# david-strejc/fei

Hardware: AMD Instinct MI355X
Metric: agent tok/s (llama3-8b local decode, 1 agent/GPU) (higher is better)
Workload: dtype bf16; 1 GPU; model=llama3-8b, global_batch=1, seq_len=512, parallelism=dp1 (1 agent per GPU, weak scaling), hip_graph=True, stream_engine=False

## Files before the change

fei_amd/models/llama.py:

```python

from __future__ import annotations

import math
import os
from dataclasses import dataclass
from typing import Dict, List, Optional

import torch
import torch.nn.functional as F

from fei_amd import ops
from fei_amd.engine.config import ModelSpec
from fei_amd.ops import reference as ref
from fei_amd.parallel.pg import ParallelContext, all_gather_cat, all_reduce_sum


@dataclass
class LayerWeights:
    norm_attn: torch.Tensor
    wqkv: torch.Tensor
    wo: torch.Tensor
    norm_mlp: torch.Tensor
    wgu: torch.Tensor
    wdown: torch.Tensor
# ... 16 lines not shown
        self.max_seq_len = max_seq_len or spec.max_seq_len
        tp_size = self.tp.world_size if self.tp.is_distributed else 1
        if spec.num_kv_heads % tp_size or spec.num_heads % tp_size or \
                spec.intermediate_size % tp_size or spec.vocab_size % tp_size:
            raise ValueError(f"model {spec.name} not divisible by tp={tp_size}")
        self.tp_size = tp_size
        self.tp_rank = self.tp.rank if self.tp.is_distributed else 0
        self.hq_l = spec.num_heads // tp_size
        self.hkv_l = spec.num_kv_heads // tp_size
        self.inter_l = spec.intermediate_size // tp_size
        self.vocab_l = spec.vocab_size // tp_size
        self.D = spec.head_dim
        self._init_weights(seed)
        self.rope = ref.rope_table(self.max_seq_len, self.D, spec.rope_theta,
                                   device=device)
        self.prefetch_mb = int(os.environ.get("FEI_PREFETCH", "0") or 0)
        self._pf_stream = None
        self._pf_sink = None
        self.norm_precomp = os.environ.get("FEI_NORM_PRECOMP", "0") == "1"


    def _rand(self, gen, *shape, scale: float) -> torch.Tensor:
        w = torch.randn(*shape, generator=gen, device=self.device,
                        dtype=torch.float32) * scale
        return w.to(self.dtype)

    def _init_weights(self, seed: int) -> None:
        s = self.spec
        gen = torch.Generator(device=self.device)
        gen.manual_seed(seed)
        C = s.hidden_size
        sc = 1.0 / math.sqrt(C)
        self.emb = self._rand(gen, s.vocab_size, C, scale=0.02)
        self.layers: List[LayerWeights] = []
        r = self.tp_rank
        for _ in range(s.num_layers):
            wq = self._rand(gen, s.num_heads * self.D, C, scale=sc)
            wk = self._rand(gen, s.num_kv_heads * self.D, C, scale=sc)
            wv = self._rand(gen, s.num_kv_heads * self.D, C, scale=sc)
            wo = self._rand(gen, C, s.num_heads * self.D, scale=sc / math.sqrt(2 * s.num_layers))
            wg = self._rand(gen, s.intermediate_size, C, scale=sc)
            wu = self._rand(gen, s.intermediate_size, C, scale=sc)
            wd = self._rand(gen, C, s.intermediate_size,
                            scale=1.0 / math.sqrt(s.intermediate_size) / math.sqrt(2 * s.num_layers))
            wq = wq.view(s.num_heads, self.D, C)[r * self.hq_l:(r + 1) * self.hq_l].reshape(-1, C)
            wk = wk.view(s.num_kv_heads, self.D, C)[r * self.hkv_l:(r + 1) * self.hkv_l].reshape(-1, C)
            wv = wv.view(s.num_kv_heads, self.D, C)[r * self.hkv_l:(r + 1) * self.hkv_l].reshape(-1, C)
            wo = wo.view(C, s.num_heads, self.D)[:, r * self.hq_l:(r + 1) * self.hq_l].reshape(C, -1)
            wg = wg[r * self.inter_l:(r + 1) * self.inter_l]
            wu = wu[r * self.inter_l:(r + 1) * self.inter_l]
            wd = wd[:, r * self.inter_l:(r + 1) * self.inter_l]
            self.layers.append(LayerWeights(
                norm_attn=torch.ones(C, device=self.device, dtype=self.dtype),
                wqkv=torch.cat([wq, wk, wv], dim=0).contiguous(),
                wo=wo.contiguous(),
                norm_mlp=torch.ones(C, device=self.device, dtype=self.dtype),
                wgu=torch.cat([wg, wu], dim=0).contiguous(),
                wdown=wd.contiguous(),
            ))
        self.norm_f = torch.ones(C, device=self.device, dtype=self.dtype)
        lm = self._rand(gen, s.vocab_size, C, scale=sc)
        self.lm_head = lm[r * self.vocab_l:(r + 1) * self.vocab_l].contiguous()
        self.vocab_offset = r * self.vocab_l

    def quantize_fp8(self) -> None:
        self.fp8 = []
        for lw in self.layers:
            self.fp8.append({
                "wqkv": ops.quant_fp8(lw.wqkv),
                "wo": ops.quant_fp8(lw.wo),
                "wgu": ops.quant_fp8(lw.wgu),
                "wdown": ops.quant_fp8(lw.wdown),
            })
        self.fp8_lm_head = ops.quant_fp8(self.lm_head)

    def param_bytes(self) -> int:
        total = self.emb.numel() + self.norm_f.numel() + self.lm_head.numel()
        for lw in self.layers:
            for t in (lw.norm_attn, lw.wqkv, lw.wo, lw.norm_mlp, lw.wgu, lw.wdown):
                total += t.numel()
        return total * self.emb.element_size()


    def new_kv_cache(self, batch: int, max_seq: Optional[int] = None,
                     kv_quant: Optional[str] = None):
        max_seq = max_seq or self.max_seq_len
        shape = (batch, self.hkv_l, max_seq, self.D)
        if kv_quant == "fp8":
            return (
                [ops.QuantKV.zeros(shape, self.device)
                 for _ in range(self.spec.num_layers)],
                [ops.QuantKV.zeros(shape, self.device)
                 for _ in range(self.spec.num_layers)],
            )
        if kv_quant is not None:
            raise ValueError(f"unknown kv_quant {kv_quant!r}")
        return (
            [torch.zeros(shape, device=self.device, dtype=self.dtype)
             for _ in range(self.spec.num_layers)],
            [torch.zeros(shape, device=self.device, dtype=self.dtype)
             for _ in range(self.spec.num_layers)],
        )


    def _qkv_views(self, qkv: torch.Tensor, B: int, S: Optional[int] = None):
        D = self.D
        W = qkv.shape[-1]
        off_k = self.hq_l * D
        off_v = off_k + self.hkv_l * D
        if S is None:
            q = qkv.as_strided((B, self.hq_l, D), (W, D, 1))
            k = qkv.as_strided((B, self.hkv_l, D), (W, D, 1), storage_offset=qkv.storage_offset() + off_k)
            v = qkv.as_strided((B, self.hkv_l, D), (W, D, 1), storage_offset=qkv.storage_offset() + off_v)
        else:
            q = qkv.as_strided((B, S, self.hq_l, D), (S * W, W, D, 1))
            k = qkv.as_strided((B, S, self.hkv_l, D), (S * W, W, D, 1), storage_offset=qkv.storage_offset() + off_k)
            v = qkv.as_strided((B, S, self.hkv_l, D), (S * W, W, D, 1), storage_offset=qkv.storage_offset() + off_v)
        return q, k, v


    def forward_decode(
        self,
        token: torch.Tensor,
        pos: torch.Tensor,
        k_caches: List[torch.Tensor],
        v_caches: List[torch.Tensor],
        attn_splits: int = 32,
        workspace=None,
        fused_attn: bool = False,
        attn_out: Optional[torch.Tensor] = None,
        fused_norm: bool = False,
        gather_logits: bool = True,
    ) -> torch.Tensor:
        if fused_norm and self.tp_size == 1 and token.shape[0] == 1 and \
                self.spec.hidden_size * 2 <= 32 * 1024:
            return self._forward_decode_fused_norm(
                token, pos, k_caches, v_caches, attn_splits, workspace,
                fused_attn, attn_out)
        s = self.spec
        B = token.shape[0]
        h = F.embedding(token.long(), self.emb)
        scale = 1.0 / math.sqrt(self.D)
        n_layers = len(self.layers)
        x = ops.rmsnorm(h, self.layers[0].norm_attn, s.norm_eps)
        addnorm = (ops._ADDNORM_GEMV and self.tp_size == 1 and B == 1
                   and h.is_cuda and h.dtype == torch.bfloat16
                   and ops._addnorm_ok(B, s.hidden_size))
        if addnorm:
            h = h.contiguous()
            hb = torch.empty(2, B, s.hidden_size, dtype=h.dtype,
                             device=h.device)
            nbuf = 0
        d = None
        for li, lw in enumerate(self.layers):
            if addnorm and li > 0:
                qkv = ops.gemv_addnorm(d, h, hb[nbuf], lw.norm_attn, lw.wqkv,
                                       s.norm_eps)
                h, nbuf = hb[nbuf], nbuf ^ 1
            else:
                qkv = ops.linear_decode(x, lw.wqkv)
            q, k, v = self._qkv_views(qkv, B)
            if fused_attn:
                att = ops.attn_decode_fused(q, k, v, k_caches[li],
                                            v_caches[li], pos, self.rope,
                                            scale=scale, out=attn_out)
            else:
                att = ops.attn_decode(q, k_caches[li], v_caches[li], pos,
                                      splits=attn_splits, scale=scale,
                                      workspace=workspace, out=attn_out,
                                      k=k, v=v, table=self.rope, layer=li)
            o = ops.linear_decode(att.reshape(B, -1), lw.wo)
            all_reduce_sum(o, self.tp)
            if addnorm:
                act = ops.gemv_swiglu_addnorm(o, h, hb[nbuf], lw.norm_mlp,
                                              lw.wgu, s.norm_eps)
                h, nbuf = hb[nbuf], nbuf ^ 1
            else:
                x, h = ops.fused_add_rmsnorm(o, h, lw.norm_mlp, s.norm_eps)
                act = ops.gemv_swiglu(x, lw.wgu)
            d = ops.linear_decode(act, lw.wdown)
            all_reduce_sum(d, self.tp)
            if addnorm and li + 1 < n_layers:
                continue
            next_norm = (self.layers[li + 1].norm_attn if li + 1 < n_layers
                         else self.norm_f)
            x, h = ops.fused_add_rmsnorm(d, h, next_norm, s.norm_eps)
        logits = ops.linear_decode(x, self.lm_head)
        if gather_logits:
            logits = all_gather_cat(logits, dim=-1, ctx=self.tp)
        return logits

    def forward_decode_stream(self, token, pos, k_caches, v_caches,
                              ws: dict, bufs) -> torch.Tensor:
        s = self.spec
        h = F.embedding(token.long(), self.emb)
        bufs[0].copy_(h.to(bufs[0].dtype))
        scale = 1.0 / math.sqrt(self.D)
        cur, nxt = bufs
        for li, lw in enumerate(self.layers):
            ops.stream_layer(cur, nxt, lw, s, k_caches[li], v_caches[li],
                             self.rope, pos, ws, li, scale)
            cur, nxt = nxt, cur
        return ops.gemv_norm(cur, self.norm_f, self.lm_head, s.norm_eps)

    def _ssq_slots(self, B: int, device) -> torch.Tensor:
        buf = getattr(self, "_ssq", None)
        if buf is None or buf.shape[1] != B or buf.device != device:
            buf = torch.zeros(2 * len(self.layers), B, dtype=torch.float32,
                              device=device)
            self._ssq = buf
        return buf

    def _forward_decode_fused_norm(self, token, pos, k_caches, v_caches,
                                   attn_splits, workspace, fused_attn,
                                   attn_out):
        s = self.spec
        B = token.shape[0]
        fp8 = getattr(self, "fp8", None)
        if fp8 is not None and (B != 1 or s.hidden_size * 2 > 32 * 1024):
            fp8 = None
        h = F.embedding(token.long(), self.emb).contiguous()
        scale = 1.0 / math.sqrt(self.D)
        ssq = (self._ssq_slots(B, h.device)
               if (self.norm_precomp and fp8 is None and h.is_cuda) else None)
        if ssq is not None:
            ssq.zero_()
        pf = self.prefetch_mb > 0 and fp8 is None and h.is_cuda
        if pf and self._pf_stream is None:
            self._pf_stream = torch.cuda.Stream()
            self._pf_sink = torch.zeros(1, dtype=torch.float32,
                                        device=h.device)
        for li, lw in enumerate(self.layers):
            if fp8 is not None:
                q8 = fp8[li]
                qkv = ops.gemv_norm_fp8(h, lw.norm_attn, *q8["wqkv"],
                                        s.norm_eps)
            else:
                qkv = ops.gemv_norm(
                    h, lw.norm_attn, lw.wqkv, s.norm_eps,
                    ssq=ssq[2 * li - 1] if (ssq is not None and li > 0) else None)
            if pf:
                ev = torch.cuda.Event()
                ev.record()
                with torch.cuda.stream(self._pf_stream):
                    self._pf_stream.wait_event(ev)
                    ops.prefetch(lw.wgu, self.prefetch_mb << 20,
                                 self._pf_sink)
            q, k, v = self._qkv_views(qkv, B)
            if fused_attn:
                att = ops.attn_decode_fused(q, k, v, k_caches[li],
                                            v_caches[li], pos, self.rope,
                                            scale=scale, out=attn_out)
            else:
                att = ops.attn_decode(q, k_caches[li], v_caches[li], pos,
                                      splits=attn_splits, scale=scale,
                                      workspace=workspace, out=attn_out,
                                      k=k, v=v, table=self.rope, layer=li)
            if fp8 is not None:
                ops.gemv_res_fp8(att.reshape(B, -1), *q8["wo"], h)
                act = ops.gemv_swiglu_norm_fp8(h, lw.norm_mlp, *q8["wgu"],
                                               s.norm_eps)
                ops.gemv_res_fp8(act, *q8["wdown"], h)
            else:
                ops.gemv_res(att.reshape(B, -1), lw.wo, h,
                             ssq_out=ssq[2 * li] if ssq is not None else None)
                act = ops.gemv_swiglu_norm(
                    h, lw.norm_mlp, lw.wgu, s.norm_eps,
                    ssq=ssq[2 * li] if ssq is not None else None)
                ops.gemv_res(act, lw.wdown, h,
                             ssq_out=ssq[2 * li + 1] if ssq is not None else None)
        if pf:
            torch.cuda.current_stream().wait_stream(self._pf_stream)
        if fp8 is not None:
            return ops.gemv_norm_fp8(h, self.norm_f, *self.fp8_lm_head,
                                     s.norm_eps)
        return ops.gemv_norm(h, self.norm_f, self.lm_head, s.norm_eps,
                             ssq=ssq[-1] if ssq is not None else None)

    def forward_prefill(
        self,
        tokens: torch.Tensor,
        pos0: torch.Tensor,
        k_caches: List[torch.Tensor],
        v_caches: List[torch.Tensor],
        all_positions: bool = False,
    ) -> torch.Tensor:
        scale = 1.0 / math.sqrt(self.D)

        def attend(li, q, k, v):
            ops.rope_kv_prefill(q, k, v, k_caches[li], v_caches[li], pos0, self.rope)
            return ops.attn_prefill(q, k_caches[li], v_caches[li], pos0, scale=scale)

        return self._prefill_layers(tokens, attend, all_positions)

    def forward_prefill_paged(
        self,
        tokens: torch.Tensor,
        pos0: torch.Tensor,
        k_pools: List[torch.Tensor],
        v_pools: List[torch.Tensor],
        block_table: torch.Tensor,
        all_positions: bool = False,
    ) -> torch.Tensor:
        if self.tp_size != 1:
            raise RuntimeError("forward_prefill_paged is single-GPU (tp=1)")
        scale = 1.0 / math.sqrt(self.D)

        def attend(li, q, k, v):
            ops.rope_kv_prefill_paged(q, k, v, k_pools[li], v_pools[li],
                                      block_table, pos0, self.rope)
            return ops.attn_prefill_paged(q, k_pools[li], v_pools[li],
                                          block_table, pos0, scale=scale)

        return self._prefill_layers(tokens, attend, all_positions)

    def _prefill_layers(self, tokens, attend, all_positions):
        s = self.spec
        B, S = tokens.shape
        h = F.embedding(tokens.long(), self.emb)
        n_layers = len(self.layers)
        x = ops.rmsnorm(h, self.layers[0].norm_attn, s.norm_eps)
        for li, lw in enumerate(self.layers):
            qkv = F.linear(x, lw.wqkv)
            qkv2 = qkv.view(B * S, -1)
            q, k, v = self._qkv_views(qkv2, B, S)
            att = attend(li, q, k, v)
            o = F.linear(att.reshape(B, S, -1), lw.wo)
            all_reduce_sum(o, self.tp)
            x, h = ops.fused_add_rmsnorm(o, h, lw.norm_mlp, s.norm_eps)
            gu = F.linear(x, lw.wgu)
            act = ops.swiglu(gu)
            d = F.linear(act, lw.wdown)
            all_reduce_sum(d, self.tp)
            next_norm = (self.layers[li + 1].norm_attn if li + 1 < n_layers
                         else self.norm_f)
            x, h = ops.fused_add_rmsnorm(d, h, next_norm, s.norm_eps)
        last = x if all_positions else x[:, -1, :]
        logits = F.linear(last, self.lm_head)
        logits = all_gather_cat(logits, dim=-1, ctx=self.tp)
        return logits
# ... 70 lines not shown
```

fei_amd/ops/__init__.py:

```python

from __future__ import annotations

import ctypes
import math
import os
from typing import Optional, Tuple

import torch

from fei_amd.ops import reference as ref

_LIB: Optional[ctypes.CDLL] = None
_LIB_ERR: Optional[str] = None
_LIB_PATH = os.path.join(os.path.dirname(os.path.abspath(__file__)),
                         "libfei_kernels.so")

_c = ctypes
_vp, _i, _f, _u64, _l = _c.c_void_p, _c.c_int, _c.c_float, _c.c_ulonglong, _c.c_long


def _try_load() -> None:
    global _LIB, _LIB_ERR
    if _LIB is not None or _LIB_ERR is not None:
        return
    try:
        lib = ctypes.CDLL(_LIB_PATH)
    except OSError as e:
        _LIB_ERR = str(e)
        return
    lib.fei_rmsnorm.argtypes = [_vp, _vp, _vp, _i, _i, _f, _vp]
    lib.fei_add_rmsnorm.argtypes = [_vp, _vp, _vp, _vp, _i, _i, _f, _vp]
    lib.fei_rope_kv_decode.argtypes = [_vp, _vp, _vp, _vp, _vp, _vp, _vp,
                                       _i, _i, _i, _i, _i, _l, _l, _vp]
    lib.fei_rope_kv_prefill.argtypes = [_vp, _vp, _vp, _vp, _vp, _vp, _vp,
                                        _i, _i, _i, _i, _i, _i, _l, _l, _vp]
    lib.fei_attn_decode.argtypes = [_vp, _vp, _vp, _vp, _vp, _vp,
                                    _i, _i, _i, _i, _i, _i, _f, _l,
                                    _vp, _vp, _vp, _l, _vp, _vp, _i, _vp]
    lib.fei_attn_decode_combine.argtypes = [_vp, _vp, _vp, _i, _i, _i, _i, _vp]
    lib.fei_swiglu.argtypes = [_vp, _vp, _l, _i, _vp]
    lib.fei_sample.argtypes = [_vp, _vp, _vp, _vp, _vp, _i, _i, _i, _f, _u64,
                               _i, _vp]
    lib.fei_advance.argtypes = [_vp, _vp, _i, _i, _vp]
    lib.fei_attn_prefill.argtypes = [_vp, _vp, _vp, _vp, _vp, _vp,
                                     _i, _i, _i, _i, _i, _i, _f, _i, _l, _vp]
    lib.fei_mfma_probe.argtypes = [_vp, _vp, _vp, _vp]
    lib.fei_gemv.argtypes = [_vp, _vp, _vp, _i, _i, _i, _i, _vp]
    lib.fei_gemm_m8.argtypes = [_vp, _vp, _vp, _i, _i, _i, _i, _vp]
    lib.fei_attn_decode_fused.argtypes = [_vp, _vp, _vp, _vp, _vp, _vp, _vp,
                                          _vp, _i, _i, _i, _i, _i, _f,
                                          _l, _l, _vp]
    lib.fei_sample_onepass.argtypes = [_vp, _vp, _vp, _vp, _i, _i, _f, _u64,
                                       _i, _vp]
    lib.fei_sample_shard.argtypes = [_vp, _vp, _vp, _i, _i, _i, _f, _u64, _vp]
    lib.fei_sample_filtered.argtypes = [_vp, _vp, _vp, _vp, _vp, _i, _i, _i,
                                        _f, _f, _u64, _i, _vp]
    lib.fei_rope_kv8_decode.argtypes = [_vp, _vp, _vp, _vp, _vp, _vp, _vp,
                                        _vp, _vp, _i, _i, _i, _i, _i, _l, _l,
                                        _vp]
    lib.fei_rope_kv8_prefill.argtypes = [_vp, _vp, _vp, _vp, _vp, _vp, _vp,
                                         _vp, _vp, _i, _i, _i, _i, _i, _i,
                                         _l, _l, _vp]
    lib.fei_attn_decode_kv8.argtypes = [_vp, _vp, _vp, _vp, _vp, _vp, _vp,
                                        _vp, _i, _i, _i, _i, _i, _i, _f, _l,
                                        _vp, _vp, _vp, _l, _vp]
    lib.fei_attn_decode_kv8.restype = _i
    lib.fei_attn_prefill_kv8.argtypes = [_vp, _vp, _vp, _vp, _vp, _vp, _vp,
                                         _i, _i, _i, _i, _i, _i, _f, _l, _vp]
    lib.fei_attn_prefill_kv8.restype = _i
    lib.fei_stream_layer_check.argtypes = [_i, _i, _i, _i, _i]
    lib.fei_stream_layer_check.restype = _i
    lib.fei_stream_layer.argtypes = [_vp, _vp, _vp, _vp, _vp, _vp, _vp, _vp,
                                     _vp, _vp, _vp, _vp, _vp, _vp, _vp, _vp,
                                     _vp, _vp, _vp, _i, _i, _i, _i, _i,
                                     _i, _i, _f, _f, _vp]
    lib.fei_attn_decode_paged.argtypes = [_vp, _vp, _vp, _vp, _vp, _vp, _vp,
                                          _i, _i, _i, _i, _i, _i, _i, _f,
                                          _l, _vp, _vp, _vp, _l, _vp]
    lib.fei_rope_kv_prefill_paged.argtypes = [_vp, _vp, _vp, _vp, _vp, _vp,
                                              _vp, _vp, _i, _i, _i, _i, _i,
                                              _i, _i, _l, _l, _vp]
    lib.fei_rope_kv_prefill_paged.restype = _i
    lib.fei_attn_prefill_paged.argtypes = [_vp, _vp, _vp, _vp, _vp, _vp,
                                           _i, _i, _i, _i, _i, _i, _i, _f,
                                           _l, _vp]
    lib.fei_attn_prefill_paged.restype = _i
    lib.fei_add_layernorm.argtypes = [_vp, _vp, _vp, _vp, _vp, _i, _i, _f,
                                      _i, _vp]
    lib.fei_gelu.argtypes = [_vp, _vp, _l, _vp]
    lib.fei_gemv_norm_fp8.argtypes = [_vp, _vp, _vp, _vp, _vp, _i, _i, _i,
                                      _f, _vp]
    lib.fei_gemv_res_fp8.argtypes = [_vp, _vp, _vp, _vp, _i, _i, _i, _vp]
    lib.fei_gemv_swiglu_norm_fp8.argtypes = [_vp, _vp, _vp, _vp, _vp, _i, _i,
                                             _i, _f, _vp]
    lib.fei_quant_fp8_rows.argtypes = [_vp, _vp, _vp, _i, _i, _vp]
    lib.fei_gemv_swiglu.argtypes = [_vp, _vp, _vp, _i, _i, _i, _i, _vp]
    lib.fei_prefetch.argtypes = [_vp, _l, _vp, _i, _vp]
    lib.fei_gemv_res.argtypes = [_vp, _vp, _vp, _i, _i, _i, _i, _vp, _vp]
    lib.fei_gemv_norm.argtypes = [_vp, _vp, _vp, _vp, _i, _i, _i, _f, _i, _vp,
                                  _vp]
    lib.fei_gemv_swiglu_norm.argtypes = [_vp, _vp, _vp, _vp, _i, _i, _i, _f,
                                         _i, _vp, _vp]
    for fn in (lib.fei_gemv_addnorm, lib.fei_gemv_swiglu_addnorm):
        fn.argtypes = [_vp, _vp, _vp, _vp, _vp, _vp, _i, _i, _i, _f, _i, _i,
                       _vp]
        fn.restype = _i
    _LIB = lib


def kernels_available() -> bool:
    _try_load()
    return _LIB is not None


def require_lib() -> ctypes.CDLL:
    _try_load()
    if _LIB is None:
        raise RuntimeError(
            "fei_amd HIP kernel library not found at "
            f"{_LIB_PATH} ({_LIB_ERR}). Build it with "
            "`python -m fei_amd.ops.build` — GPU execution refuses to fall "
            "back to eager PyTorch.")
    return _LIB


def _stream() -> int:
    return torch.cuda.current_stream().cuda_stream


def _ptr(t: torch.Tensor) -> int:
    return t.data_ptr()




class QuantKV:

    __slots__ = ("data", "scale")

    def __init__(self, data: torch.Tensor, scale: torch.Tensor):
        assert data.dtype == torch.uint8 and scale.dtype == torch.float32
        assert tuple(scale.shape) == tuple(data.shape[:-1])
        assert data.is_contiguous() and scale.is_contiguous(), \
            "QuantKV needs contiguous data and scale"
        assert data.data_ptr() % 16 == 0, "QuantKV data must be 16 B aligned"
        self.data = data
        self.scale = scale

    @classmethod
    def zeros(cls, shape, device) -> "QuantKV":
        return cls(torch.zeros(shape, dtype=torch.uint8, device=device),
                   torch.ones(shape[:-1], dtype=torch.float32, device=device))

    @property
    def shape(self):
        return self.data.shape

    def dequant(self, length: Optional[int] = None) -> torch.Tensor:
        n = self.data.shape[2] if length is None else length
        return ref.dequant_kv_fp8(self.data[:, :, :n], self.scale[:, :, :n])


def _kv8_pair(k_cache, v_cache) -> bool:
    k8, v8 = isinstance(k_cache, QuantKV), isinstance(v_cache, QuantKV)
    if k8 != v8:
        raise TypeError("k_cache and v_cache must both be QuantKV or both "
                        "be tensors")
    return k8


def _check_gqa(name: str, Hq: int, Hkv: int) -> None:
    if Hkv <= 0 or Hq % Hkv != 0 or Hq // Hkv not in (1, 2, 4, 8):
        raise ValueError(f"{name}: unsupported GQA group Hq={Hq}, Hkv={Hkv} "
                         "(Hq/Hkv must be 1, 2, 4 or 8)")


def _check_vec8(name: str, n: int, what: str = "last dimension") -> None:
    if n % 8 != 0:
        raise ValueError(f"{name}: {what} must be a multiple of 8, got {n}")


def rmsnorm(x: torch.Tensor, weight: torch.Tensor, eps: float = 1e-5,
            out: Optional[torch.Tensor] = None) -> torch.Tensor:
    _check_vec8("rmsnorm", x.shape[-1])
    if x.numel() == 0:
        return torch.empty_like(x) if out is None else out
    if not x.is_cuda:
        return ref.rmsnorm(x, weight, eps)
    lib = require_lib()
    x2 = x.contiguous()
    if out is None:
        out = torch.empty_like(x2)
    rows = x2.numel() // x2.shape[-1]
    lib.fei_rmsnorm(_ptr(out), _ptr(x2), _ptr(weight), rows, x2.shape[-1],
                    eps, _stream())
    return out


def fused_add_rmsnorm(x: torch.Tensor, residual: torch.Tensor,
                      weight: torch.Tensor, eps: float = 1e-5,
                      out: Optional[torch.Tensor] = None
                      ) -> Tuple[torch.Tensor, torch.Tensor]:
    _check_vec8("fused_add_rmsnorm", x.shape[-1])
    if not residual.is_contiguous():
        raise ValueError("fused_add_rmsnorm: residual must be contiguous "
                         "(it is updated in place)")
    if x.numel() == 0:
        return (torch.empty_like(x) if out is None else out), residual
    if not x.is_cuda:
        o, res = ref.fused_add_rmsnorm(x, residual, weight, eps)
        residual.copy_(res)
        return o, residual
    lib = require_lib()
    x2 = x.contiguous()
    if out is None:
        out = torch.empty_like(x2)
    rows = x2.numel() // x2.shape[-1]
    lib.fei_add_rmsnorm(_ptr(out), _ptr(residual), _ptr(x2), _ptr(weight),
                        rows, x2.shape[-1], eps, _stream())
    return out, residual


def rope_kv_decode(q, k, v, k_cache, v_cache, pos, table) -> torch.Tensor:
    kv8 = _kv8_pair(k_cache, v_cache)
    if not q.is_cuda:
        if kv8:
            q_out = ref.rope_kv_decode_fp8(
                q, k, v, k_cache.data, k_cache.scale, v_cache.data,
                v_cache.scale, pos, table)
        else:
            q_out = ref.rope_kv_decode(q, k, v, k_cache, v_cache, pos, table)
        q.copy_(q_out)
        return q
    lib = require_lib()
    B, Hq, D = q.shape
    Hkv = k.shape[1]
    assert q.stride(2) == 1 and q.stride(1) == D, "head rows must be contiguous"
    assert k.stride(1) == D and v.stride(1) == D
    assert k.stride(0) == v.stride(0)
    if kv8:
        assert D in (64, 128), f"fp8 KV append supports D in (64,128), got {D}"
        lib.fei_rope_kv8_decode(_ptr(q), _ptr(k), _ptr(v), _ptr(k_cache.data),
                                _ptr(k_cache.scale), _ptr(v_cache.data),
                                _ptr(v_cache.scale), _ptr(table), _ptr(pos),
                                B, Hq, Hkv, D, k_cache.shape[2],
                                q.stride(0), k.stride(0), _stream())
        return q
    lib.fei_rope_kv_decode(_ptr(q), _ptr(k), _ptr(v), _ptr(k_cache),
                           _ptr(v_cache), _ptr(table), _ptr(pos),
                           B, Hq, Hkv, D, k_cache.shape[2],
                           q.stride(0), k.stride(0), _stream())
    return q


def rope_kv_prefill(q, k, v, k_cache, v_cache, pos0, table) -> torch.Tensor:
    kv8 = _kv8_pair(k_cache, v_cache)
    if not q.is_cuda:
        if kv8:
            q_out = ref.rope_kv_prefill_fp8(
# ... 242 lines not shown
    if out is None:
        out = torch.empty(*gu.shape[:-1], inter, dtype=gu.dtype, device=gu.device)
    lib.fei_swiglu(_ptr(out), _ptr(gu), rows, inter, _stream())
    return out


def sample(logits: torch.Tensor, token: torch.Tensor,
           step: torch.Tensor, workspace: torch.Tensor,
           out_tokens: Optional[torch.Tensor] = None,
           temperature: float = 0.0, seed: int = 0,
           nchunks: int = 64) -> torch.Tensor:
    B, V = logits.shape
    if not logits.is_cuda:
        if temperature <= 0:
            t = ref.argmax_sample(logits)
        else:
            g = torch.Generator().manual_seed(
                (int(seed) * 1000003 + int(step)) & 0x7FFFFFFF)
            t = ref.gumbel_sample(logits, temperature, g)
        token.copy_(t)
        if out_tokens is not None:
            st = int(step)
            for b in range(B):
                if st < out_tokens.shape[1]:
                    out_tokens[b, st] = t[b]
        return token
    lib = require_lib()
    max_new = out_tokens.shape[1] if out_tokens is not None else 0
    out_ptr = _ptr(out_tokens) if out_tokens is not None else None
    if B <= 8:
        lib.fei_sample_onepass(_ptr(logits), _ptr(token), out_ptr, _ptr(step),
                               B, V, temperature, seed, max_new, _stream())
    else:
        lib.fei_sample(_ptr(logits), _ptr(token), out_ptr, _ptr(step),
                       _ptr(workspace), B, V, nchunks, temperature, seed,
                       max_new, _stream())
    return token


def sample_filtered(logits: torch.Tensor, token: torch.Tensor,
                    step: torch.Tensor, info: torch.Tensor,
                    out_tokens: Optional[torch.Tensor] = None,
                    temperature: float = 0.0, seed: int = 0,
                    top_k: int = 0, top_p: float = 1.0) -> torch.Tensor:
    if top_k < 0:
        raise ValueError(f"top_k must be >= 0, got {top_k}")
    if not 0.0 < top_p <= 1.0:
        raise ValueError(f"top_p must be in (0, 1], got {top_p}")
    B, V = logits.shape
    if not logits.is_cuda:
        keep, thr, count = ref.filter_keep(logits, top_k, top_p)
        info[:, 0] = thr
        info[:, 1].view(torch.int32).copy_(count)
        if keep.all():
            masked = logits
        else:
            masked = logits.float().masked_fill(~keep, float("-inf"))
        return sample(masked, token, step, None, out_tokens=out_tokens,
                      temperature=temperature, seed=seed)
    lib = require_lib()
    max_new = out_tokens.shape[1] if out_tokens is not None else 0
    out_ptr = _ptr(out_tokens) if out_tokens is not None else None
    lib.fei_sample_filtered(_ptr(logits), _ptr(token), out_ptr, _ptr(step),
                            _ptr(info), B, V, int(top_k), float(top_p),
                            float(temperature), int(seed), max_new, _stream())
    return token


def sample_shard(logits: torch.Tensor, step: torch.Tensor,
                 v_offset: int, out: torch.Tensor,
                 temperature: float = 0.0, seed: int = 0) -> torch.Tensor:
    B, Vl = logits.shape
    if not logits.is_cuda:
        vals = logits.float()
        if temperature > 0:
            vals = vals / temperature + ref.hash_gumbel(
                B, Vl, v_offset, int(seed), int(step))
        best = vals.max(dim=-1)
        out[:, 0] = best.values
        out[:, 1].view(torch.int32).copy_(
            (best.indices + v_offset).to(torch.int32))
        return out
    lib = require_lib()
    lib.fei_sample_shard(_ptr(logits), _ptr(out), _ptr(step), B, Vl,
                         int(v_offset), float(temperature), int(seed),
                         _stream())
    return out



STREAM_NSPLIT = 32


def stream_layer_check(C: int, Hq: int, Hkv: int, D: int, I: int) -> int:
    lib = require_lib()
    return int(lib.fei_stream_layer_check(C, Hq, Hkv, D, I))


def stream_workspace(spec, device) -> dict:
    C, D = spec.hidden_size, spec.head_dim
    Hq, Hkv, I = spec.num_heads, spec.num_kv_heads, spec.intermediate_size
    mk = lambda n: torch.zeros(n, dtype=torch.int64, device=device)
    return {
        "g_qkv": mk((Hq + 2 * Hkv) * D),
        "g_att": mk(Hq * D // 2),
        "g_h2": mk(C // 2),
        "g_act": mk(I),
        "g_done": mk(6 * 256),
        "fail": torch.zeros(1, dtype=torch.int32, device=device),
    }


def stream_layer(x_in: torch.Tensor, h_out: torch.Tensor, lw, spec,
                 k_cache: torch.Tensor, v_cache: torch.Tensor,
                 cos_sin: torch.Tensor, pos: torch.Tensor, ws: dict,
                 layer: int, scale: float) -> None:
    lib = require_lib()
    lib.fei_stream_layer(
        _ptr(x_in), _ptr(h_out), _ptr(lw.wqkv), _ptr(lw.wo), _ptr(lw.wgu),
        _ptr(lw.wdown), _ptr(lw.norm_attn), _ptr(lw.norm_mlp),
        _ptr(k_cache), _ptr(v_cache), _ptr(cos_sin), _ptr(pos),
        _ptr(ws["g_qkv"]), _ptr(ws["g_att"]),
        _ptr(ws["g_h2"]), _ptr(ws["g_act"]), _ptr(ws["g_done"]),
        _ptr(ws["dbg"]) if "dbg" in ws else None,
        _ptr(ws["fail"]),
        spec.hidden_size, spec.num_heads, spec.num_kv_heads, spec.head_dim,
        spec.intermediate_size, k_cache.shape[-2], layer, spec.norm_eps,
        scale, _stream())


def advance(pos: torch.Tensor, step: torch.Tensor,
            max_pos: int = 1 << 30) -> None:
    if not pos.is_cuda:
        pos.clamp_(max=max_pos - 1)
        pos += 1
        step += 1
        return
    lib = require_lib()
    lib.fei_advance(_ptr(pos), _ptr(step), pos.shape[0], max_pos, _stream())


def mfma_probe(A: torch.Tensor, B: torch.Tensor) -> torch.Tensor:
    lib = require_lib()
    C = torch.empty(16, 16, dtype=torch.float32, device=A.device)
    lib.fei_mfma_probe(_ptr(A.contiguous()), _ptr(B.contiguous()), _ptr(C),
                       _stream())
    return C



_GEMV_NT_MIN_BYTES = int(os.environ.get("FEI_GEMV_NT_MIN", 0))
_FUSED_CMB = os.environ.get("FEI_FUSED_CMB", "0") == "1"
_ADDNORM_GEMV = os.environ.get("FEI_ADDNORM_GEMV", "1") == "1"


def _gemm_m8_ok(M: int, N: int, K: int) -> bool:
    return 4 <= M <= 8 and K % 1024 == 0 and N % 16 == 0


def _gemv_ok(M: int, K: int) -> bool:
    return M in (1, 2, 4, 8) and K % 8 == 0


def linear_decode(x: torch.Tensor, w: torch.Tensor,
                  out: Optional[torch.Tensor] = None) -> torch.Tensor:
    M = x.numel() // x.shape[-1]
    K = x.shape[-1]
    N = w.shape[0]
    if not x.is_cuda or not (_gemv_ok(M, K) or _gemm_m8_ok(M, N, K)):
        return torch.nn.functional.linear(x, w)
    lib = require_lib()
    x2 = x.contiguous().view(M, K)
    if out is None:
        out = torch.empty(*x.shape[:-1], N, dtype=x.dtype, device=x.device)
    nt = 1 if (N * K * 2 >= _GEMV_NT_MIN_BYTES) else 0
    if _gemm_m8_ok(M, N, K):
        lib.fei_gemm_m8(_ptr(out), _ptr(x2), _ptr(w), M, N, K, 0,
                        _stream())
        return out
    lib.fei_gemv(_ptr(out), _ptr(x2), _ptr(w), M, N, K, nt, _stream())
    return out


def gemv_swiglu(x: torch.Tensor, wgu: torch.Tensor,
                out: Optional[torch.Tensor] = None) -> torch.Tensor:
    M = x.numel() // x.shape[-1]
    K = x.shape[-1]
    I = wgu.shape[0] // 2
    if not x.is_cuda:
        return ref.swiglu(torch.nn.functional.linear(x, wgu))
    if not (_gemv_ok(M, K) or _gemm_m8_ok(M, 2 * I, K)):
        return swiglu(torch.nn.functional.linear(x, wgu))
    lib = require_lib()
    x2 = x.contiguous().view(M, K)
    if out is None:
        out = torch.empty(*x.shape[:-1], I, dtype=x.dtype, device=x.device)
    nt = 1 if (2 * I * K * 2 >= _GEMV_NT_MIN_BYTES) else 0
    if _gemm_m8_ok(M, 2 * I, K):
        gu = torch.empty(M, 2 * I, dtype=x.dtype, device=x.device)
        lib.fei_gemm_m8(_ptr(gu), _ptr(x2), _ptr(wgu), M, 2 * I, K, 0,
                        _stream())
        lib.fei_swiglu(_ptr(out), _ptr(gu), M, I, _stream())
        return out
    lib.fei_gemv_swiglu(_ptr(out), _ptr(x2), _ptr(wgu), M, I, K, nt,
                        _stream())
    return out


def gemv_res(x: torch.Tensor, w: torch.Tensor, res: torch.Tensor,
             ssq_out: Optional[torch.Tensor] = None) -> torch.Tensor:
    M = x.numel() // x.shape[-1]
    K = x.shape[-1]
    N = w.shape[0]
    if not x.is_cuda or not _gemv_ok(M, K):
        lin = torch.nn.functional.linear(x, w)
        res.copy_((res.float() + lin.float().view_as(res)).to(res.dtype))
        return res
    lib = require_lib()
    x2 = x.contiguous().view(M, K)
    nt = 1 if (N * K * 2 >= _GEMV_NT_MIN_BYTES) else 0
    lib.fei_gemv_res(_ptr(res), _ptr(x2), _ptr(w), M, N, K, nt,
                     _ptr(ssq_out) if ssq_out is not None else None,
                     _stream())
    return res


def gemv_norm(res: torch.Tensor, wnorm: torch.Tensor, w: torch.Tensor,
              eps: float = 1e-5,
              out: Optional[torch.Tensor] = None,
              ssq: Optional[torch.Tensor] = None) -> torch.Tensor:
    M = res.numel() // res.shape[-1]
    K = res.shape[-1]
    N = w.shape[0]
    if not res.is_cuda or not _gemv_ok(M, K):
        return torch.nn.functional.linear(rmsnorm(res, wnorm, eps), w)
    lib = require_lib()
    r2 = res.contiguous().view(M, K)
    if out is None:
        out = torch.empty(*res.shape[:-1], N, dtype=res.dtype, device=res.device)
    nt = 1 if (N * K * 2 >= _GEMV_NT_MIN_BYTES) else 0
    lib.fei_gemv_norm(_ptr(out), _ptr(r2), _ptr(wnorm), _ptr(w), M, N, K,
                      eps, nt, _ptr(ssq) if ssq is not None else None,
                      _stream())
    return out


def gemv_swiglu_norm(res: torch.Tensor, wnorm: torch.Tensor,
                     wgu: torch.Tensor, eps: float = 1e-5,
                     out: Optional[torch.Tensor] = None,
                     ssq: Optional[torch.Tensor] = None) -> torch.Tensor:
    M = res.numel() // res.shape[-1]
    K = res.shape[-1]
    I = wgu.shape[0] // 2
    if not res.is_cuda or not _gemv_ok(M, K):
        gu = torch.nn.functional.linear(rmsnorm(res, wnorm, eps).float(),
                                        wgu.float())
        return ref.swiglu(gu).to(res.dtype)
    lib = require_lib()
    r2 = res.contiguous().view(M, K)
    if out is None:
        out = torch.empty(*res.shape[:-1], I, dtype=res.dtype, device=res.device)
    nt = 1 if (wgu.shape[0] * K * 2 >= _GEMV_NT_MIN_BYTES) else 0
    lib.fei_gemv_swiglu_norm(_ptr(out), _ptr(r2), _ptr(wnorm), _ptr(wgu),
                             M, I, K, eps, nt,
                             _ptr(ssq) if ssq is not None else None,
                             _stream())
    return out



_ADDNORM_ROW_GROUPS = max(1, int(os.environ.get("FEI_ADDNORM_RG", "2") or 2))
_ADDNORM_ROW_GROUPS_SWIGLU = max(
    1, int(os.environ.get("FEI_ADDNORM_RG_SWIGLU", "2") or 2))


def _addnorm_ok(M: int, K: int) -> bool:
    return M == 1 and _gemv_ok(M, K) and M * K * 2 <= 32 * 1024


def _addnorm_check(name: str, delta, res_in, res_out) -> None:
    if not res_in.is_contiguous() or not res_out.is_contiguous():
        raise ValueError(f"{name}: res_in and res_out must be contiguous")
    if res_in.shape != res_out.shape or res_in.dtype != res_out.dtype:
        raise ValueError(f"{name}: res_in and res_out must match in shape "
                         "and dtype")
    if delta.shape != res_in.shape:
        raise ValueError(f"{name}: delta must have the residual's shape")
    a0, b0 = res_in.data_ptr(), res_out.data_ptr()
    nbytes = res_in.numel() * res_in.element_size()
    if a0 < b0 + nbytes and b0 < a0 + nbytes:
        raise ValueError(f"{name}: res_in and res_out must not share storage "
                         "(the new residual cannot be written in place)")


def gemv_addnorm(delta: torch.Tensor, res_in: torch.Tensor,
                 res_out: torch.Tensor, wnorm: torch.Tensor, w: torch.Tensor,
                 eps: float = 1e-5,
                 out: Optional[torch.Tensor] = None) -> torch.Tensor:
    _addnorm_check("gemv_addnorm", delta, res_in, res_out)
    K = res_in.shape[-1]
    M = res_in.numel() // max(K, 1)
    N = w.shape[0]
    if not res_in.is_cuda or not _addnorm_ok(M, K):
        res_out.copy_(res_in)
        x, _ = fused_add_rmsnorm(delta, res_out, wnorm, eps)
        return linear_decode(x, w, out=out)
    lib = require_lib()
    d2 = delta.contiguous()
    if out is None:
        out = torch.empty(*res_in.shape[:-1], N, dtype=res_in.dtype,
                          device=res_in.device)
    nt = 1 if (N * K * 2 >= _GEMV_NT_MIN_BYTES) else 0
    rc = lib.fei_gemv_addnorm(_ptr(out), _ptr(d2), _ptr(res_in),
                              _ptr(res_out), _ptr(wnorm), _ptr(w), M, N, K,
                              eps, nt, _ADDNORM_ROW_GROUPS, _stream())
    if rc != 0:
        raise RuntimeError(f"fei_gemv_addnorm refused the launch (rc={rc})")
    return out


def gemv_swiglu_addnorm(delta: torch.Tensor, res_in: torch.Tensor,
                        res_out: torch.Tensor, wnorm: torch.Tensor,
                        wgu: torch.Tensor, eps: float = 1e-5,
                        out: Optional[torch.Tensor] = None) -> torch.Tensor:
    _addnorm_check("gemv_swiglu_addnorm", delta, res_in, res_out)
    K = res_in.shape[-1]
    M = res_in.numel() // max(K, 1)
    I = wgu.shape[0] // 2
    if not res_in.is_cuda or not _addnorm_ok(M, K):
        res_out.copy_(res_in)
        x, _ = fused_add_rmsnorm(delta, res_out, wnorm, eps)
# ... 297 lines not shown
```

fei_amd/ops/csrc/gemv.hip:

```cpp
#include "fei_common.h"

namespace {

template <int M, bool NT>
__global__ void __launch_bounds__(256)
k_gemv(u16* __restrict__ out, const u16* __restrict__ x,
       const u16* __restrict__ w, int N, int K) {
  const int tid = threadIdx.x;
  const int lane = tid & 63;
  const int wid = tid >> 6;
  const int n0 = blockIdx.x * 8 + wid * 2;
  if (n0 >= N) return;
  const u16* xs = x;
  const bool two = (n0 + 1) < N;

  const s16x8* wrow0 = (const s16x8*)(w + (long)n0 * K);
  const s16x8* wrow1 = (const s16x8*)(w + (long)(n0 + (two ? 1 : 0)) * K);
  float acc0[M], acc1[M];
#pragma unroll
  for (int m = 0; m < M; ++m) { acc0[m] = 0.f; acc1[m] = 0.f; }
  const int nv = K >> 3;
  for (int i = lane; i < nv; i += 64) {
    s16x8 wv0, wv1;
    if (NT) {
      wv0 = __builtin_nontemporal_load(&wrow0[i]);
      wv1 = __builtin_nontemporal_load(&wrow1[i]);
    } else {
      wv0 = wrow0[i];
      wv1 = wrow1[i];
    }
#pragma unroll
    for (int m = 0; m < M; ++m) {
      s16x8 xv = ((const s16x8*)(xs + m * K))[i];
      acc0[m] += dot8_bf16(xv, wv0);
      acc1[m] += dot8_bf16(xv, wv1);
    }
  }
#pragma unroll
  for (int m = 0; m < M; ++m) {
    float v0 = wave_reduce_sum(acc0[m]);
    float v1 = wave_reduce_sum(acc1[m]);
    if (lane == 0) {
      out[(long)m * N + n0] = f2bf(v0);
      if (two) out[(long)m * N + n0 + 1] = f2bf(v1);
    }
  }
}

template <int M, bool NT>
__global__ void __launch_bounds__(256)
k_gemv_swiglu(u16* __restrict__ out, const u16* __restrict__ x,
              const u16* __restrict__ w, int N, int K) {
  const int tid = threadIdx.x;
  const int lane = tid & 63;
  const int wid = tid >> 6;
  const int n = blockIdx.x * 4 + wid;
  if (n >= N) return;
  const u16* xs = x;

  const s16x8* grow = (const s16x8*)(w + (long)n * K);
  const s16x8* urow = (const s16x8*)(w + (long)(n + N) * K);
  float accg[M], accu[M];
#pragma unroll
  for (int m = 0; m < M; ++m) { accg[m] = 0.f; accu[m] = 0.f; }
  const int nv = K >> 3;
  for (int i = lane; i < nv; i += 64) {
    s16x8 gv = NT ? __builtin_nontemporal_load(&grow[i]) : grow[i];
    s16x8 uv = NT ? __builtin_nontemporal_load(&urow[i]) : urow[i];
#pragma unroll
    for (int m = 0; m < M; ++m) {
      s16x8 xv = ((const s16x8*)(xs + m * K))[i];
      accg[m] += dot8_bf16(xv, gv);
      accu[m] += dot8_bf16(xv, uv);
    }
  }
#pragma unroll
  for (int m = 0; m < M; ++m) {
    float g = wave_reduce_sum(accg[m]);
    float u = wave_reduce_sum(accu[m]);
    if (lane == 0) {
      const float silu = g / (1.f + __expf(-g));
      out[(long)m * N + n] = f2bf(silu * u);
    }
  }
}

}

extern "C" {

void fei_gemv(void* out, const void* x, const void* w, int M, int N, int K,
              int nontemporal, hipStream_t stream) {
  dim3 grid((N + 7) / 8);
  const size_t lds = 0;
#define LG(MV, NTV) hipLaunchKernelGGL((k_gemv<MV, NTV>), grid, dim3(256), \
                                       lds, stream, (u16*)out, \
                                       (const u16*)x, (const u16*)w, N, K)
#define LGD(MV) do { if (nontemporal) LG(MV, true); else LG(MV, false); } while (0)
  switch (M) {
    case 1: LGD(1); break;
    case 2: LGD(2); break;
    case 4: LGD(4); break;
    case 8: LGD(8); break;
    default: break;
  }
#undef LGD
#undef LG
}

void fei_gemv_swiglu(void* out, const void* x, const void* w, int M, int N,
                     int K, int nontemporal, hipStream_t stream) {
  dim3 grid((N + 3) / 4);
  const size_t lds = 0;
#define LG(MV, NTV) hipLaunchKernelGGL((k_gemv_swiglu<MV, NTV>), grid, \
                                  dim3(256), lds, stream, (u16*)out, \
                                  (const u16*)x, (const u16*)w, N, K)
#define LGD(MV) do { if (nontemporal) LG(MV, true); else LG(MV, false); } while (0)
  switch (M) {
    case 1: LGD(1); break;
    case 2: LGD(2); break;
    case 4: LGD(4); break;
    case 8: LGD(8); break;
    default: break;
  }
#undef LGD
#undef LG
}

}


namespace {

template <int M>
__device__ __forceinline__ void norm_factors(const u16* __restrict__ res,
                                             int K, float eps, int lane,
                                             float inv[M]) {
#pragma unroll
  for (int m = 0; m < M; ++m) {
    const s16x8* row = (const s16x8*)(res + (long)m * K);
    float ss = 0.f;
    const int nv = K >> 3;
    for (int i = lane; i < nv; i += 64) {
      s16x8 v = row[i];
#pragma unroll
      for (int j = 0; j < 8; ++j) {
        const float f = bf2f((u16)v[j]);
        ss = fmaf(f, f, ss);
      }
    }
    ss = wave_reduce_sum(ss);
    inv[m] = rsqrtf(ss / (float)K + eps);
  }
}

template <int M, bool NT>
__global__ void __launch_bounds__(256)
k_gemv_res(u16* __restrict__ res, const u16* __restrict__ x,
           const u16* __restrict__ w, int N, int K, float* __restrict__ ssq) {
  const int tid = threadIdx.x;
  const int lane = tid & 63;
  const int wid = tid >> 6;
  const int n0 = blockIdx.x * 8 + wid * 2;
  const bool active = n0 < N;
  const bool two = (n0 + 1) < N;
  const s16x8* wrow0 = (const s16x8*)(w + (long)(active ? n0 : 0) * K);
  const s16x8* wrow1 = (const s16x8*)(w + (long)(active ? n0 + (two ? 1 : 0) : 0) * K);
  float acc0[M], acc1[M], mysq[M];
#pragma unroll
  for (int m = 0; m < M; ++m) { acc0[m] = 0.f; acc1[m] = 0.f; mysq[m] = 0.f; }
  const int nv = K >> 3;
  if (active) {
    for (int i = lane; i < nv; i += 64) {
      s16x8 wv0 = NT ? __builtin_nontemporal_load(&wrow0[i]) : wrow0[i];
      s16x8 wv1 = NT ? __builtin_nontemporal_load(&wrow1[i]) : wrow1[i];
#pragma unroll
      for (int m = 0; m < M; ++m) {
        s16x8 xv = ((const s16x8*)(x + (long)m * K))[i];
        acc0[m] += dot8_bf16(xv, wv0);
        acc1[m] += dot8_bf16(xv, wv1);
      }
    }
  }
#pragma unroll
  for (int m = 0; m < M; ++m) {
    const float v0 = wave_reduce_sum(acc0[m]);
    const float v1 = wave_reduce_sum(acc1[m]);
    if (lane == 0 && active) {
      u16* r = res + (long)m * N + n0;
      const u16 b0 = f2bf(bf2f(r[0]) + v0);
      r[0] = b0;
      const float f0 = bf2f(b0);
      mysq[m] = f0 * f0;
      if (two) {
        const u16 b1 = f2bf(bf2f(r[1]) + v1);
        r[1] = b1;
        const float f1 = bf2f(b1);
        mysq[m] += f1 * f1;
      }
    }
  }
  if (ssq) {
    __shared__ float sred[4][M];
    if (lane == 0) {
#pragma unroll
      for (int m = 0; m < M; ++m) sred[wid][m] = mysq[m];
    }
    __syncthreads();
    if (tid == 0) {
#pragma unroll
      for (int m = 0; m < M; ++m)
        atomicAdd(&ssq[m], sred[0][m] + sred[1][m] + sred[2][m] + sred[3][m]);
    }
  }
}

template <int M, bool NT>
__global__ void __launch_bounds__(256)
k_gemv_norm(u16* __restrict__ out, const u16* __restrict__ res,
            const u16* __restrict__ wn, const u16* __restrict__ w,
            int N, int K, float eps, const float* __restrict__ ssq) {
  const int tid = threadIdx.x;
  const int lane = tid & 63;
  const int wid = tid >> 6;
  const int n0 = blockIdx.x * 8 + wid * 2;
  if (n0 >= N) return;
  float inv[M];
  if (ssq) {
#pragma unroll
    for (int m = 0; m < M; ++m)
      inv[m] = rsqrtf(ssq[m] / (float)K + eps);
  } else {
    norm_factors<M>(res, K, eps, lane, inv);
  }
  const bool two = (n0 + 1) < N;
  const s16x8* wrow0 = (const s16x8*)(w + (long)n0 * K);
  const s16x8* wrow1 = (const s16x8*)(w + (long)(n0 + (two ? 1 : 0)) * K);
  float acc0[M], acc1[M];
#pragma unroll
  for (int m = 0; m < M; ++m) { acc0[m] = 0.f; acc1[m] = 0.f; }
  const int nv = K >> 3;
  for (int i = lane; i < nv; i += 64) {
    s16x8 wv0 = NT ? __builtin_nontemporal_load(&wrow0[i]) : wrow0[i];
    s16x8 wv1 = NT ? __builtin_nontemporal_load(&wrow1[i]) : wrow1[i];
    s16x8 wnv = ((const s16x8*)wn)[i];
#pragma unroll
    for (int m = 0; m < M; ++m) {
      s16x8 xv = ((const s16x8*)(res + (long)m * K))[i];
#pragma unroll
      for (int j = 0; j < 8; ++j) {
        const float xn = bf2f(f2bf(bf2f((u16)xv[j]) * inv[m] * bf2f((u16)wnv[j])));
        acc0[m] = fmaf(xn, bf2f((u16)wv0[j]), acc0[m]);
        acc1[m] = fmaf(xn, bf2f((u16)wv1[j]), acc1[m]);
      }
    }
  }
#pragma unroll
  for (int m = 0; m < M; ++m) {
    const float v0 = wave_reduce_sum(acc0[m]);
    const float v1 = wave_reduce_sum(acc1[m]);
    if (lane == 0) {
      out[(long)m * N + n0] = f2bf(v0);
      if (two) out[(long)m * N + n0 + 1] = f2bf(v1);
    }
  }
}

template <int M, bool NT>
__global__ void __launch_bounds__(256)
k_gemv_swiglu_norm(u16* __restrict__ out, const u16* __restrict__ res,
                   const u16* __restrict__ wn, const u16* __restrict__ w,
                   int N, int K, float eps, const float* __restrict__ ssq) {
  const int tid = threadIdx.x;
  const int lane = tid & 63;
  const int wid = tid >> 6;
  const int n = blockIdx.x * 4 + wid;
  if (n >= N) return;
  float inv[M];
  if (ssq) {
// ... 196 lines not shown
```

Measured before the change: 312.1 tok/s.

## Add deep register-ring GEMV for M=1 decode with small grids

Adds a new M=1 GEMV kernel that keeps an 8-deep ring of x and weight vector loads in registers per lane. Each step consumes one slot and refills it with the load 8 steps ahead, and the trip count is unrolled as a template parameter. linear_decode picks this path on a single GPU when the grid is small relative to the CU count, so more memory requests are in flight per wave when there are too few waves to hide latency. The cost is much higher register use, which lowers occupancy, and a clamped index that loads past-the-end elements redundantly. On MI355X, the llama3-8b wo, wdown and qkv projections (N of 4096 or 6144) fall under the threshold.

After: 329.7 tok/s, median of 6. 5.7% higher.

```diff
diff --git a/fei_amd/models/llama.py b/fei_amd/models/llama.py
--- a/fei_amd/models/llama.py
+++ b/fei_amd/models/llama.py
@@ -192,13 +192,14 @@
                              device=h.device)
             nbuf = 0
         d = None
+        deep = None if self.tp_size == 1 else False
         for li, lw in enumerate(self.layers):
             if addnorm and li > 0:
                 qkv = ops.gemv_addnorm(d, h, hb[nbuf], lw.norm_attn, lw.wqkv,
                                        s.norm_eps)
                 h, nbuf = hb[nbuf], nbuf ^ 1
             else:
-                qkv = ops.linear_decode(x, lw.wqkv)
+                qkv = ops.linear_decode(x, lw.wqkv, deep=deep)
             q, k, v = self._qkv_views(qkv, B)
             if fused_attn:
                 att = ops.attn_decode_fused(q, k, v, k_caches[li],
@@ -209,7 +210,7 @@
                                       splits=attn_splits, scale=scale,
                                       workspace=workspace, out=attn_out,
                                       k=k, v=v, table=self.rope, layer=li)
-            o = ops.linear_decode(att.reshape(B, -1), lw.wo)
+            o = ops.linear_decode(att.reshape(B, -1), lw.wo, deep=deep)
             all_reduce_sum(o, self.tp)
             if addnorm:
                 act = ops.gemv_swiglu_addnorm(o, h, hb[nbuf], lw.norm_mlp,
@@ -218,14 +219,14 @@
             else:
                 x, h = ops.fused_add_rmsnorm(o, h, lw.norm_mlp, s.norm_eps)
                 act = ops.gemv_swiglu(x, lw.wgu)
-            d = ops.linear_decode(act, lw.wdown)
+            d = ops.linear_decode(act, lw.wdown, deep=deep)
             all_reduce_sum(d, self.tp)
             if addnorm and li + 1 < n_layers:
                 continue
             next_norm = (self.layers[li + 1].norm_attn if li + 1 < n_layers
                          else self.norm_f)
             x, h = ops.fused_add_rmsnorm(d, h, next_norm, s.norm_eps)
-        logits = ops.linear_decode(x, self.lm_head)
+        logits = ops.linear_decode(x, self.lm_head, deep=deep)
         if gather_logits:
             logits = all_gather_cat(logits, dim=-1, ctx=self.tp)
         return logits
diff --git a/fei_amd/ops/__init__.py b/fei_amd/ops/__init__.py
--- a/fei_amd/ops/__init__.py
+++ b/fei_amd/ops/__init__.py
@@ -105,6 +105,8 @@
         fn.argtypes = [_vp, _vp, _vp, _vp, _vp, _vp, _i, _i, _i, _f, _i, _i,
                        _vp]
         fn.restype = _i
+    lib.fei_gemv_deep.argtypes = [_vp, _vp, _vp, _i, _i, _i, _i, _vp]
+    lib.fei_gemv_deep.restype = _i
     _LIB = lib
 
 
@@ -653,6 +655,11 @@
 _GEMV_NT_MIN_BYTES = int(os.environ.get("FEI_GEMV_NT_MIN", 0))
 _FUSED_CMB = os.environ.get("FEI_FUSED_CMB", "0") == "1"
 _ADDNORM_GEMV = os.environ.get("FEI_ADDNORM_GEMV", "1") == "1"
+_GEMV_DEEP = os.environ.get("FEI_GEMV_DEEP", "1") == "1"
+_GEMV_DEEP_MAX_WG_PER_CU = float(
+    os.environ.get("FEI_GEMV_DEEP_MAX_WG_PER_CU", "8") or 8)
+_GEMV_DEEP_MAX_TRIPS = 8
+_CU_COUNT: dict = {}
 
 
 def _gemm_m8_ok(M: int, N: int, K: int) -> bool:
@@ -663,8 +670,28 @@
     return M in (1, 2, 4, 8) and K % 8 == 0
 
 
+def _cu_count(device: torch.device) -> int:
+    idx = device.index if device.index is not None else \
+        torch.cuda.current_device()
+    if idx not in _CU_COUNT:
+        _CU_COUNT[idx] = torch.cuda.get_device_properties(
+            idx).multi_processor_count
+    return _CU_COUNT[idx]
+
+
+def _gemv_deep_ok(M: int, K: int) -> bool:
+    return (M == 1 and K > 0 and K % 8 == 0
+            and -(-K // 4096) <= _GEMV_DEEP_MAX_TRIPS)
+
+
+def _gemv_deep_wins(N: int, K: int, device: torch.device) -> bool:
+    return (_GEMV_DEEP and _gemv_deep_ok(1, K)
+            and (N + 7) // 8 < _GEMV_DEEP_MAX_WG_PER_CU * _cu_count(device))
+
+
 def linear_decode(x: torch.Tensor, w: torch.Tensor,
-                  out: Optional[torch.Tensor] = None) -> torch.Tensor:
+                  out: Optional[torch.Tensor] = None,
+                  deep: Optional[bool] = None) -> torch.Tensor:
     M = x.numel() // x.shape[-1]
     K = x.shape[-1]
     N = w.shape[0]
@@ -678,6 +705,15 @@
     if _gemm_m8_ok(M, N, K):
         lib.fei_gemm_m8(_ptr(out), _ptr(x2), _ptr(w), M, N, K, 0,
                         _stream())
+        return out
+    if deep is None:
+        deep = M == 1 and _gemv_deep_wins(N, K, x.device)
+    if deep:
+        rc = lib.fei_gemv_deep(_ptr(out), _ptr(x2), _ptr(w), M, N, K, nt,
+                               _stream())
+        if rc != 0:
+            raise ValueError(
+                f"gemv_deep does not take M={M} N={N} K={K} (code {rc})")
         return out
     lib.fei_gemv(_ptr(out), _ptr(x2), _ptr(w), M, N, K, nt, _stream())
     return out
diff --git a/fei_amd/ops/csrc/gemv.hip b/fei_amd/ops/csrc/gemv.hip
--- a/fei_amd/ops/csrc/gemv.hip
+++ b/fei_amd/ops/csrc/gemv.hip
@@ -125,6 +125,119 @@
   }
 #undef LGD
 #undef LG
+}
+
+}
+
+
+namespace {
+
+template <bool NT>
+__device__ __forceinline__ s16x8 ldw_deep(const s16x8* p) {
+  return NT ? __builtin_nontemporal_load(p) : *p;
+}
+
+template <int D, bool NT, bool REFILL>
+__device__ __forceinline__ void deep_ring(float& acc0, float& acc1,
+                                          s16x8 (&xv)[D], s16x8 (&wv0)[D],
+                                          s16x8 (&wv1)[D],
+                                          const s16x8* __restrict__ xr,
+                                          const s16x8* __restrict__ wrow0,
+                                          const s16x8* __restrict__ wrow1,
+                                          int base, int nv, int lane) {
+#pragma unroll
+  for (int u = 0; u < D; ++u) {
+    const int i = base + u * 64 + lane;
+    const float d0 = dot8_bf16(xv[u], wv0[u]);
+    const float d1 = dot8_bf16(xv[u], wv1[u]);
+    acc0 = i < nv ? acc0 + d0 : acc0;
+    acc1 = i < nv ? acc1 + d1 : acc1;
+    if (REFILL) {
+      const int j = min(i + D * 64, nv - 1);
+      xv[u] = xr[j];
+      wv0[u] = ldw_deep<NT>(&wrow0[j]);
+      wv1[u] = ldw_deep<NT>(&wrow1[j]);
+    }
+    __builtin_amdgcn_sched_barrier(0);
+  }
+}
+
+template <int D, bool NT, int T>
+__global__ void __launch_bounds__(256)
+k_gemv_deep(u16* __restrict__ out, const u16* __restrict__ x,
+            const u16* __restrict__ w, int N, int K) {
+  const int tid = threadIdx.x;
+  const int lane = tid & 63;
+  const int wid = tid >> 6;
+  const int n0 = blockIdx.x * 8 + wid * 2;
+  if (n0 >= N) return;
+  const bool two = (n0 + 1) < N;
+  const s16x8* xr = (const s16x8*)x;
+  const s16x8* wrow0 = (const s16x8*)(w + (long)n0 * K);
+  const s16x8* wrow1 = (const s16x8*)(w + (long)(n0 + (two ? 1 : 0)) * K);
+  const int nv = K >> 3;
+
+  s16x8 xv[D], wv0[D], wv1[D];
+#pragma unroll
+  for (int u = 0; u < D; ++u) xv[u] = xr[min(lane + u * 64, nv - 1)];
+#pragma unroll
+  for (int u = 0; u < D; ++u) {
+    const int j = min(lane + u * 64, nv - 1);
+    wv0[u] = ldw_deep<NT>(&wrow0[j]);
+    wv1[u] = ldw_deep<NT>(&wrow1[j]);
+  }
+  __builtin_amdgcn_sched_barrier(0);
+
+  float acc0 = 0.f, acc1 = 0.f;
+#pragma unroll
+  for (int t = 0; t < T - 1; ++t)
+    deep_ring<D, NT, true>(acc0, acc1, xv, wv0, wv1, xr, wrow0, wrow1,
+                           t * D * 64, nv, lane);
+  deep_ring<D, NT, false>(acc0, acc1, xv, wv0, wv1, xr, wrow0, wrow1,
+                          (T - 1) * D * 64, nv, lane);
+
+  const float v0 = wave_reduce_sum(acc0);
+  const float v1 = wave_reduce_sum(acc1);
+  if (lane == 0) {
+    out[n0] = f2bf(v0);
+    if (two) out[n0 + 1] = f2bf(v1);
+  }
+}
+
+}
+
+extern "C" {
+
+#define FEI_GEMV_DEEP_RING 8
+#define FEI_GEMV_DEEP_MAX_TRIPS 8
+int fei_gemv_deep(void* out, const void* x, const void* w, int M, int N,
+                  int K, int nontemporal, hipStream_t stream) {
+  if (M != 1) return -1;
+  if (K <= 0 || K % 8 != 0 || N < 1) return -2;
+  const int per_trip = FEI_GEMV_DEEP_RING * 64;
+  const int trips = ((K >> 3) + per_trip - 1) / per_trip;
+  if (trips > FEI_GEMV_DEEP_MAX_TRIPS) return -2;
+  dim3 grid((N + 7) / 8);
+#define LD(TV) do { \
+    if (nontemporal) \
+      hipLaunchKernelGGL((k_gemv_deep<FEI_GEMV_DEEP_RING, true, TV>), grid, \
+          dim3(256), 0, stream, (u16*)out, (const u16*)x, (const u16*)w, N, K); \
+    else \
+      hipLaunchKernelGGL((k_gemv_deep<FEI_GEMV_DEEP_RING, false, TV>), grid, \
+          dim3(256), 0, stream, (u16*)out, (const u16*)x, (const u16*)w, N, K); \
+  } while (0)
+  switch (trips) {
+    case 1: LD(1); break;
+    case 2: LD(2); break;
+    case 3: LD(3); break;
+    case 4: LD(4); break;
+    case 5: LD(5); break;
+    case 6: LD(6); break;
+    case 7: LD(7); break;
+    default: LD(8); break;
+  }
+#undef LD
+  return 0;
 }
 
 }
```
